# nidium/libapenetwork

Hardware: AMD Instinct MI355X
Metric: LZ4 GiB/s device-resident (compress+decompress), 1M×64KiB blocks, 1/2/4/8 GPU (higher is better)
Workload: dtype u8

## Files before the change

### libapenetwork_amd/csrc/lz4_encode.hip

```cpp
#include "lz4_gpu_internal.h"
#include <type_traits>

namespace apelz4 {

#ifdef APE_LZ4_STATS
__device__ unsigned long long g_enc_stats[16];
hipError_t enc_stats_read(unsigned long long *out, int reset) {
    hipError_t e = hipMemcpyFromSymbol(out, HIP_SYMBOL(g_enc_stats), sizeof(g_enc_stats));
    if (e == hipSuccess && reset) {
        unsigned long long z[16] = {0};
        e = hipMemcpyToSymbol(HIP_SYMBOL(g_enc_stats), z, sizeof(z));
    }
    return e;
}
#endif

namespace {

constexpr int kWavesPerEu = 7;

constexpr uint32_t kEagerLen = 12;
static_assert(kEagerLen + 4u == 16u, "in[T-4, T+kEagerLen) is one 16-byte load (loadv)");
constexpr uint32_t kEagerL = 12;
constexpr uint32_t kExt2 = 64;
constexpr uint32_t kGroups = 16;
constexpr uint32_t kRingE = 1024;
static_assert((kRingE & (kRingE - 1u)) == 0u && kRingE < 65536u,
              "the ring holds recent input, not the block's window (DESIGN.md 3.1.1)");
constexpr int kSmall = 128;
constexpr uint32_t kQ = 128;
constexpr uint32_t kFetchAt = 48, kEmitAll = 80, kChunkRecs = 64u / 4u;
static_assert((kQ & (kQ - 1u)) == 0u, "record ring indexed by & (kQ - 1)");
static_assert(kEmitAll - 1u + 2u * kChunkRecs <= kQ, "walker -> emitter record ring overflow");
static_assert(kFetchAt < kEmitAll, "a fetch precedes emit_all");
constexpr int kEmitEvery = 8;
constexpr uint32_t kStage = 512;
constexpr uint32_t kStageAlloc = kStage + 16u + 16u + 64u;


constexpr uint32_t I_TRUNC = 1u << 7, I_HASHABLE = 1u << 13;
static_assert(kEagerLen + kExt2 < 128u, "len fits 7 bits");

struct __attribute__((aligned(16))) EncLds {
    uint32_t ring[kRingE / 4 + 16];
    uint16_t tab[kHSize];
    uint2 info[64];
    uint2 q[kQ];
    uint32_t qn[2];
    uint8_t __attribute__((aligned(16))) stage[kStageAlloc];
};

template <int N>
__device__ __forceinline__ void vm_wait() {
    static_assert(N >= 0 && N < 16, "vmcnt");
    __builtin_amdgcn_s_waitcnt(N | (7 << 4) | (15 << 8));
}

__device__ __forceinline__ void shift_bytes(const uint32_t (&L)[8], int d, uint32_t (&X)[8]) {
    uint32_t T[8];
#pragma unroll
    for (int k = 0; k < 8; k++) T[k] = L[k];
    const bool down = d >= 0;
    const int ad = down ? d : -d, w = ad >> 2;
    const uint32_t r = (uint32_t)ad & 3u;
#pragma unroll
    for (int bit = 4; bit >= 1; bit >>= 1) {
        if (w & bit) {
            if (down) {
#pragma unroll
                for (int k = 0; k < 8; k++) T[k] = (k + bit < 8) ? T[k + bit] : 0u;
            } else {
#pragma unroll
                for (int k = 7; k >= 0; k--) T[k] = (k - bit >= 0) ? T[k - bit] : 0u;
            }
        }
    }
#pragma unroll
    for (int k = 0; k < 8; k++) {
        if (down) X[k] = __builtin_amdgcn_alignbyte(k + 1 < 8 ? T[k + 1] : 0u, T[k], r);
        else X[k] = r ? __builtin_amdgcn_alignbyte(T[k], k >= 1 ? T[k - 1] : 0u, 4u - r) : T[k];
    }
}

// ... 135 lines not shown
    int nch;
    int k0;
    uint32_t nr;
    uint32_t stride;
    gcu8 *win;
    uint32_t D;
};

template <bool EXT>
__device__ __forceinline__ gcu8 *hist(const Blk &B, uint32_t pos) {
    if constexpr (EXT) return pos < B.D ? B.win + pos : B.in + pos;
    else return B.in + pos;
}
template <bool EXT, int NA>
__device__ __forceinline__ void loadv_h(const Blk &B, uint32_t pos, uint32_t (&X)[NA], bool fast) {
    if constexpr (!EXT) {
        loadv(B.in, B.un, pos, X, fast);
    } else {
        gcu8 *q = hist<true>(B, pos);
        if (fast) {
            const uint4 a = gload16(q);
            X[0] = a.x; X[1] = a.y; X[2] = a.z; X[3] = a.w;
            return;
        }
#pragma unroll
        for (int k = 0; k < 4; k++) X[k] = 0;
#pragma unroll
        for (uint32_t t = 0; t < 16u; t++)
            if (pos + t < B.un) X[t >> 2] |= (uint32_t)q[t] << (8 * (t & 3));
    }
}

struct Part {
    uint32_t len, c, bk, lim, base;
    uint32_t iy;
    uint32_t rank, ntr, eo;
    bool hashable;
    uint64_t tmask;
    uint64_t smask;
};

struct PSet {
    uint32_t X[2];
    uint32_t Y[6];
    uint32_t E[4];
    uint32_t cT, jL, h;
    Part q;
};

template <bool SMALL, bool FAST = false, bool EXT = false>
__device__ __forceinline__ void prod_load(const Blk &B, int k, int lane, uint32_t (&X)[2]) {
    const uint32_t pos = (FAST || k < B.nch ? 64u * (uint32_t)k : (EXT ? B.D : 0u)) + (uint32_t)lane;
    if (FAST || (!SMALL && 64 * k + 72 <= B.n)) {
        const uint2 v = gload8(B.in + pos);
        X[0] = v.x;
        X[1] = v.y;
        return;
    }
    X[0] = X[1] = 0;
#pragma unroll
    for (uint32_t t = 0; t < 8u; t++)
        if (pos + t < B.un) X[t >> 2] |= (uint32_t)B.in[pos + t] << (8 * (t & 3));
}

template <bool SMALL, bool FAST = false, bool EXT = false>
__device__ __forceinline__ void prod_fetch_t(const Blk &B, int k, int lane, uint32_t cT,
                                             uint32_t (&Y)[6]) {
    const uint32_t p = 64u * (uint32_t)k + (uint32_t)lane;
    if (FAST) {
        loadv_h<EXT>(B, __builtin_elementwise_sub_sat(umin(cT, p - 1u), 4u), Y, true);
        return;
    }
    const bool tryT = k < B.nch && cT < p && cT >= 4u;
    loadv_h<EXT>(B, tryT ? cT - 4u : 0u, Y, !SMALL && 64 * k + 83 <= B.n);
}

template <bool SMALL, bool FAST = false, bool EXT = false>
__device__ __forceinline__ void prod_lookup(EncLds &S, const Blk &B, int k, int lane,
                                            const uint32_t (&X)[2], uint32_t &cT, uint32_t &jL,
                                            uint32_t &h, uint32_t (&Y)[6]) {
    const uint32_t p = 64u * (uint32_t)k + (uint32_t)lane;
    const bool hashable = FAST || (k < B.nch && p + 5u <= B.un);
    h = hashk(X[0], X[1]);
    cT = S.tab[h];
    jL = 0xFFFFFFFFu;
    if (hashable) S.tab[h] = (uint16_t)p;
    prod_fetch_t<SMALL, FAST, EXT>(B, k, lane, cT, Y);
}

template <bool FAST = false>
__device__ __forceinline__ void prod_ring(EncLds &S, const Blk &B, int k, int lane,
                                          const uint32_t (&X)[2]) {
    if (FAST || k < B.nch) {
        const uint32_t p = 64u * (uint32_t)k + (uint32_t)lane;
        const uint8_t by = (uint8_t)X[0];
        ((uint8_t *)S.ring)[p & (kRingE - 1)] = by;
        if (((64u * (uint32_t)k) & (kRingE - 1)) == 0u) ((uint8_t *)S.ring)[kRingE + lane] = by;
    }
}

__device__ __forceinline__ void prod_own(const EncLds &S, int k, int lane, uint32_t (&X)[6]) {
    const uint32_t p = 64u * (uint32_t)k + (uint32_t)lane;
    const uint32_t *r = S.ring + (((p - 4u) >> 2) & (kRingE / 4 - 1));
    const uint32_t sh = p & 3u;
    uint32_t W[7];
#pragma unroll
    for (int t = 0; t < 7; t++) W[t] = r[t];
#pragma unroll
    for (int t = 0; t < 6; t++) X[t] = __builtin_amdgcn_alignbyte(W[t + 1], W[t], sh);
}

__device__ __forceinline__ bool stage2_group(const Part &R, int lane, uint32_t first, uint32_t p,
                                             uint32_t &cb, uint32_t &eo) {
    const uint32_t r = R.rank - first, i16 = 16u * ((uint32_t)lane & 3u);
    const bool push = lane_in(R.smask) && r < kGroups;
    const int tgt = (int)((push ? 4u * r : ((uint32_t)lane | 1u)) << 2);
    cb = dpp_z<0x00>((uint32_t)__builtin_amdgcn_ds_permute(tgt, (int)(R.c + R.base))) + i16;
    eo = dpp_z<0x00>((uint32_t)__builtin_amdgcn_ds_permute(tgt, (int)(p + R.base))) + i16;
    return first + ((uint32_t)lane >> 2) < R.ntr;
}

__device__ __forceinline__ uint32_t stage2_len(const EncLds &S, int lane, uint32_t eo,
                                               const uint32_t (&E)[4]) {
    const uint4 o = ring16(S, eo);
    const uint32_t O[4] = {o.x, o.y, o.z, o.w};
    const uint32_t li = 128u * ((uint32_t)lane & 3u);
    uint32_t d = umin(first_diff_bit<0>(O, E), 8u * kExt2 - li) + li;
    d = umin(d, dpp<0xB1>(0u, d));
    d = umin(d, dpp<0x4E>(0u, d));
    const uint32_t len = d >> 3;
    return eo + len;
}

template <bool SMALL, bool FAST = false, bool EXT = false>
__device__ __forceinline__ void prod_measure(EncLds &S, const Blk &B, int k, int lane,
                                             const uint32_t (&X)[6], const uint32_t (&Y)[6],
                                             uint32_t cT, uint32_t jL, uint32_t h, Part &R) {
    const uint32_t p = 64u * (uint32_t)k + (uint32_t)lane;
    const bool live = FAST || k < B.nch;
    R.hashable = FAST || (live && p + 5u <= B.un);
    const bool can = FAST || (live && p >= 1u && p <= B.mstart && B.n >= kMinLength);
    const uint32_t cL = 64u * (uint32_t)k + jL;
    uint32_t Z[4];
#pragma unroll
    for (int t = 0; t < 4; t++) Z[t] = bperm(X[t], jL);
    constexpr bool okL = false;
    const bool okT = can & (cT < p) & (cT >= 4u) & (Y[1] == X[1]) & (!EXT | (cT + 3u - B.D > 6u));
    R.lim = FAST ? 0xFFFFu : (can ? B.mlimit - p : 0u);
    if constexpr (EXT) R.lim = cT < B.D ? umin(R.lim, B.D - cT) : R.lim;
    const uint32_t eT = eager(X, Y);
    const uint32_t eL = (umin(first_diff_bit<2>(X, Z), 8u * (kEagerL - 4u)) >> 3) + 4u;
    const uint32_t lT = okT ? eT : 0u, lL = okL ? eL : 0u;
    const bool pickL = okL & (!okT | ((lT < kEagerL) & (lL >= lT)));
    R.c = pickL ? cL : cT;
    R.len = pickL ? lL : lT;
    R.base = pickL ? kEagerL : kEagerLen;
    if (FAST && !EXT) {
        R.tmask = wave_ballot(R.len >= R.base);
    } else {
        R.tmask = wave_ballot(R.len >= R.base) & wave_ballot(R.lim > R.base);
        R.len = umin(R.len, R.lim);
    }
    {
        const uint32_t key = (R.c - (uint32_t)lane) + (R.base << 24);
        const uint32_t keyn = dpp_z<kDppWaveShl1>(key);
        R.smask = R.tmask & ~((R.tmask >> 1) & wave_ballot(key == keyn));
    }
    R.bk = umin(back4(X[0], pickL ? Z[0] : Y[0]), R.c);
    R.iy = ((okT | okL) ? p - R.c : 0u) | (h << 16);
}

template <bool SMALL, bool FAST = false, bool EXT = false>
__device__ __forceinline__ void prod_stage2_issue(const EncLds &S, const Blk &B, int k, int lane,
                                                  Part &R, uint32_t (&E)[4]) {
    const uint32_t p = 64u * (uint32_t)k + (uint32_t)lane;
    const uint64_t tb = R.smask;
    R.ntr = (uint32_t)__popcll(tb);
    R.rank = lane_rank(tb);
    uint32_t cb;
    const bool ga = stage2_group(R, lane, 0u, p, cb, R.eo);
    loadv_h<EXT>(B, ga ? cb : 0u, E, FAST || (!SMALL && 64 * k + 148 <= B.n));
}

template <bool SMALL, bool FAST = false, bool EXT = false>
__device__ __forceinline__ void prod_finish(EncLds &S, const Blk &B, int k, int lane,
                                            const Part &R, const uint32_t (&E)[4]) {
    const uint32_t p = 64u * (uint32_t)k + (uint32_t)lane;
    uint32_t len = R.len;
    bool trunc = false;
    {
        uint32_t mine = bperm(stage2_len(S, lane, R.eo, E), 4u * R.rank);
        for (uint32_t first = kGroups; first < R.ntr; first += kGroups) {
            uint32_t cb, eo, E2[4];
            const bool ga = stage2_group(R, lane, first, p, cb, eo);
            loadv_h<EXT>(B, ga ? cb : 0u, E2, FAST || (!SMALL && 64 * k + 148 <= B.n));
            const uint32_t m2 = bperm(stage2_len(S, lane, eo, E2), 4u * (R.rank - first));
            if (R.rank - first < kGroups) mine = m2;
        }
        if (lane_in(R.tmask)) {
            const uint32_t cap = R.base + kExt2, full = mine - p;
            len = (FAST && !EXT) ? umin(full, cap) : umin(umin(full, cap), R.lim);
            trunc = full >= cap && ((FAST && !EXT) || R.lim > cap);
        }
    }
    S.info[lane] = make_uint2(len | (R.bk << 8) | (trunc ? I_TRUNC : 0u) |
                                  ((FAST || R.hashable) ? I_HASHABLE : 0u),
                              R.iy);
}

struct Walk {
    uint32_t q;
    uint32_t anchor;
};

struct Probe {
    uint32_t s0, s1, g0;
};
__device__ __forceinline__ Probe probe_regime(uint32_t P, uint32_t e0, uint32_t acc) {
    const uint32_t y0 = P > e0 + 2u ? P - e0 - 2u : 0u;
    uint32_t s = 0, g = acc;
    while (y0 > s + 64u * g) {
        s += 64u * g;
        g++;
    }
    Probe R;
    R.s0 = s;
    R.s1 = s + 64u * g;
    R.g0 = g;
    return R;
}
__device__ __forceinline__ bool probed(uint32_t d, bool far, const Probe &R, uint32_t acc) {
    const uint32_t y = d - 2u;
    const bool hi = far && y > R.s1;
    const uint32_t base = far ? (hi ? R.s1 : R.s0) : 0u;
    const uint32_t g = far ? (hi ? R.g0 + 1u : R.g0) : acc;
    return d <= 2u || (y - base) % g == 0u;
}

template <bool EXT = false>
__device__ __forceinline__ uint32_t extend_match(const Blk &B, uint32_t m, uint32_t cm, uint32_t L,
// ... 9 lines not shown
                const uint4 x = gload16(B.in + (m + kk)), y = gload16(hist<EXT>(B, cm + kk));
                xb[0] = x.x; xb[1] = x.y; xb[2] = x.z; xb[3] = x.w;
                yb[0] = y.x; yb[1] = y.y; yb[2] = y.z; yb[3] = y.w;
            } else {
#pragma unroll
                for (uint32_t t = 0; t < 16u; t++) {
                    if (m + kk + t < B.un) {
                        xb[t >> 2] |= (uint32_t)B.in[m + kk + t] << (8 * (t & 3));
                        yb[t >> 2] |= (uint32_t)*hist<EXT>(B, cm + kk + t) << (8 * (t & 3));
                    }
                }
            }
#pragma unroll
            for (int t = 3; t >= 0; t--) {
                const uint32_t e = xb[t] ^ yb[t];
                if (e) { d = 1; at = 4u * (uint32_t)t + (__builtin_ctz(e) >> 3); }
            }
        }
        const uint64_t bad = wave_ballot(d != 0 || kk >= lm);
        if (bad) {
            const int fl = __builtin_ctzll(bad);
            const uint32_t k2 = L + 16u * (uint32_t)fl;
            L = k2 >= lm ? lm : k2 + lane_val(at, fl);
            break;
        }
        L += 1024u;
    }
    return L > lm ? lm : L;
}

struct WalkOut {
    uint64_t members;
    uint32_t m_back, m_len, an;
    uint2 iv;
    uint32_t q0, Lf;
    uint2 e2v;
    uint32_t e2h;
    uint32_t pmv, pe;
};

#pragma clang diagnostic push
#pragma clang diagnostic ignored "-Winline-asm"
__device__ __forceinline__ void hop_chain(uint64_t Hm, uint32_t nxt, uint32_t &rel, uint64_t &M, uint32_t &j,
                                          uint32_t &pe, uint32_t &pmv) {
    uint64_t t;
    asm volatile(
        "1:\n\t"
        "s_lshr_b64 %[t], %[hm], %[rel]\n\t"
        "s_cmp_eq_u64 %[t], 0\n\t"
        "s_cbranch_scc1 2f\n\t"
        "s_ff1_i32_b64 %[j], %[t]\n\t"
        "s_add_u32 %[j], %[j], %[rel]\n\t"
        "s_bitset1_b64 %[m], %[j]\n\t"
        "s_mov_b32 m0, %[j]\n\t"
        "v_writelane_b32 %[pmv], %[pe], m0\n\t"
        "v_readlane_b32 %[rel], %[nxt], %[j]\n\t"
        "s_mov_b32 %[pe], %[rel]\n\t"
        "s_cmp_lt_u32 %[rel], 64\n\t"
        "s_cbranch_scc1 1b\n\t"
        "s_branch 3f\n"
        "2:\n\t"
        "s_mov_b32 %[rel], 64\n"
        "3:"
        : [rel] "+s"(rel), [m] "+s"(M), [j] "+s"(j), [t] "=&s"(t), [pe] "+s"(pe), [pmv] "+v"(pmv)
        : [hm] "s"(Hm), [nxt] "v"(nxt)
        : "scc", "m0");
}
#pragma clang diagnostic pop

template <bool ACC, bool EXT = false>
__device__ __forceinline__ void walk_chain(const EncLds &S, const Blk &B, int k, int lane, Walk &W,
                                           WalkOut &O) {
    const uint32_t P = 64u * (uint32_t)k;
    O.members = 0;
    O.m_back = O.m_len = O.an = 0;
    O.iv = S.info[lane];
    O.q0 = W.q;
    O.pe = W.anchor - P;
    O.Lf = O.iv.x & 0x7Fu;
    if (W.q >= P + 64u) return;
    const uint2 iv = O.iv;
    const uint64_t Hm = wave_ballot(O.Lf != 0u);
    const uint32_t Lh = iv.x & 0xFFu;
    uint32_t rel = W.q - P;
    uint64_t M = 0;
    if constexpr (!ACC) {
        const uint32_t nxt = (uint32_t)lane + (iv.x & 0x7Fu) + ((iv.x & 0x80u) << 1);
        uint32_t j = 0;
        hop_chain(Hm, nxt, rel, M, j, O.pe, O.pmv);
        while (__builtin_expect(rel >= 256u, 0)) {
            const uint32_t me = P + j;
            const uint32_t cm = me - (lane_val(iv.y, (int)j) & 0xFFFFu);
            const uint32_t Le = extend_match<EXT>(B, me, cm, rel - 256u - j, lane);
            if ((uint32_t)lane == j) O.Lf = Le;
            rel = j + Le;
            O.pe = rel;
            if (rel >= 64u) break;
            hop_chain(Hm, nxt, rel, M, j, O.pe, O.pmv);
        }
        O.members = M;
        W.q = P + rel;
        return;
    }
    const Probe R = probe_regime(P, W.anchor, B.stride);
    uint32_t e = W.anchor;
    bool far = true;
    for (;;) {
        const uint32_t x = P + (uint32_t)lane;
        const uint64_t pm = wave_ballot(x >= e && probed(x - e, far, R, B.stride));
        const uint64_t w = (Hm & pm) >> rel;
        if (w == 0) {
            rel = 64u;
            break;
        }
        const uint32_t j = rel + (uint32_t)__builtin_ctzll(w);
        const uint32_t h = lane_val(Lh, (int)j);
        M |= 1ull << j;
        if (h & 0x80u) {
            const uint32_t me = P + j;
            const uint32_t cm = me - (lane_val(iv.y, (int)j) & 0xFFFFu);
            const uint32_t Le = extend_match<EXT>(B, me, cm, h & 0x7Fu, lane);
            if ((uint32_t)lane == j) O.Lf = Le;
            rel = j + Le;
        } else {
            rel = j + h;
        }
        e = P + rel;
        far = false;
        if (rel >= 64u) break;
    }
    O.members = M;
    W.q = P + rel;
}

template <bool ACC>
__device__ __forceinline__ void walk_finish(const Blk &B, int k, int lane, Walk &W, WalkOut &O) {
    const uint32_t P = 64u * (uint32_t)k;
    const uint32_t anchor0 = W.anchor;
    const bool mem = lane_in(O.members);
    const uint32_t p = P + (uint32_t)lane;
    uint32_t pm, lastend;
    if constexpr (!ACC) {
        pm = P + O.pmv;
        lastend = P + O.pe;
    } else {
        const uint32_t end = mem ? p + O.Lf : 0u;
        const uint32_t imax = wave_incl_max(end);
        pm = umax(wave_shr1(imax, 0u), anchor0);
        lastend = umax(anchor0, lane_val(imax, 63));
    }
    uint32_t bk = umin((O.iv.x >> 8) & 7u, p - pm);
    if (ACC) {
        const uint32_t c = p - (O.iv.y & 0xFFFFu);
        const uint32_t room = umin(p - pm, c);
        if (mem && bk == 4u && room > 4u) {
            const uint32_t lim = umin(room - 4u, 16u);
            uint32_t more = 0;
            for (uint32_t t = 1; t <= lim; t++) {
                if (B.in[p - 4u - t] != B.in[c - 4u - t]) break;
                more = t;
            }
            bk += more;
        }
    }
    O.m_back = bk;
    O.m_len = O.Lf + bk;
    O.an = pm;
    W.anchor = lastend;
}

__device__ __forceinline__ void walk_publish(EncLds &S, const Blk &B, int k, int lane,
                                             const WalkOut &O, uint32_t &qn) {
    const uint32_t p = 64u * (uint32_t)k + (uint32_t)lane;
    const uint2 iv = O.iv;
    const bool mem = lane_in(O.members);
    if (mem) S.q[(qn + lane_rank(O.members)) & (kQ - 1u)] =
        make_uint2(((p - O.m_back) - O.an) | ((O.m_len - kMinMatch) << 16), iv.y & 0xFFFFu);
    qn += (uint32_t)__popcll(O.members);
    if (lane == 0) S.qn[0] = qn;
}

struct Emit {
    uint32_t o;
    uint32_t ein;
    uint32_t qc;
    int last;
    bool overflow;
    bool part;
    int pend;
    bool nv;
    uint32_t o0, tot;
    uint64_t bigm;
    uint32_t r, lit, mlm4, off, ba;
};

__device__ __forceinline__ void stage_put(EncLds &S, int lane, bool w, uint32_t at, uint32_t b) {
    S.stage[w ? at : kStageAlloc - 64u + (uint32_t)lane] = (uint8_t)b;
}

__device__ __forceinline__ void emit_fetch(EncLds &S, const Blk &B, int lane, Emit &E,
                                           uint32_t avail, uint32_t rlo) {
    const bool v0 = (uint32_t)lane < avail;
    const uint2 rec = S.q[(E.qc + (uint32_t)lane) & (kQ - 1u)];
    const uint32_t lit = v0 ? (rec.x & 0xFFFFu) : 0u, mlm4 = v0 ? (rec.x >> 16) : 0u;
    const uint32_t size = v0 ? 3u + ext_bytes(lit) + lit + ext_bytes(mlm4) : 0u;
    const uint32_t isz = wave_incl_sum(size);
    const uint32_t nrec = umax((uint32_t)__popcll(wave_ballot(v0) & wave_ballot(isz <= kStage)), 1u);
    const bool v = (uint32_t)lane < nrec;
    const uint32_t adv = v ? lit + mlm4 + kMinMatch : 0u;
    const uint32_t iadv = wave_incl_sum(adv);
    const uint32_t tot = lane_val(isz, (int)nrec - 1), tadv = lane_val(iadv, (int)nrec - 1);
    E.qc += nrec;
// ... 123 lines not shown
        uint2 x[kU];
        bool ok[kU];
#pragma unroll
        for (int u = 0; u < kU; u++) {
            const uint32_t v = v0 + 192u * u + 3u * (uint32_t)lane;
            ok[u] = v < D && v + 8u <= B.un;
            x[u] = gload8(B.in + (ok[u] ? v : 0u));
        }
#pragma unroll
        for (int u = 0; u < kU; u++) {
            const uint32_t v = v0 + 192u * u + 3u * (uint32_t)lane;
            if (ok[u]) S.tab[hashk(x[u].x, x[u].y)] = (uint16_t)v;
        }
    }
    const uint32_t p = D - 64u + (uint32_t)lane;
    const uint8_t by = B.in[p];
    ((uint8_t *)S.ring)[p & (kRingE - 1)] = by;
    if (((D - 64u) & (kRingE - 1)) == 0u) ((uint8_t *)S.ring)[kRingE + lane] = by;
}

__device__ __forceinline__ void cdict_history(EncLds &S, const Blk &B, int lane) {
    const uint32_t p = B.D - 64u + (uint32_t)lane;
    const uint8_t by = B.win[p];
    ((uint8_t *)S.ring)[p & (kRingE - 1)] = by;
    if (((B.D - 64u) & (kRingE - 1)) == 0u) ((uint8_t *)S.ring)[kRingE + lane] = by;
}

template <bool SMALL, bool ACC, bool EXT = false>
__device__ __forceinline__ void encode_block(EncLds &S, const Blk &B, int wave, int lane,
                                             int *result, int *tail) {
    STATS_DECL
    const int k0 = B.k0;
    const int nch = B.nr >= (uint32_t)kMinLength ? B.nch : k0;
    const int nsteps = k0 + ((nch - k0 + 3) & ~1);

    if (wave == 1) {
        PSet P0, P1;
        auto pstep = [&](auto fast, int s, PSet &cur, PSet &nxt) {
            constexpr bool F = decltype(fast)::value;
            vm_wait<3>();
            STAT(9);
            prod_ring<F>(S, B, s + 2, lane, cur.X);
            uint32_t X6[6];
            prod_own(S, s + 1, lane, X6);
            prod_lookup<SMALL, F, EXT>(S, B, s + 2, lane, cur.X, cur.cT, cur.jL, cur.h, cur.Y);
            prod_load<SMALL, F, EXT>(B, s + 4, lane, cur.X);
            STAT(5);
            vm_wait<4>();
            STAT(9);
            prod_measure<SMALL, F, EXT>(S, B, s + 1, lane, X6, nxt.Y, nxt.cT, nxt.jL, nxt.h, nxt.q);
            STAT(5);
            __syncthreads();
            STAT(6);
            prod_stage2_issue<SMALL, F, EXT>(S, B, s + 1, lane, nxt.q, nxt.E);
            STAT(7);
            vm_wait<3>();
            STAT(9);
            prod_finish<SMALL, F, EXT>(S, B, s, lane, cur.q, cur.E);
            STAT(7);
            __syncthreads();
            STAT(8);
        };
        if constexpr (EXT) {
            if (k0 > 0) cdict_history(S, B, lane);
        } else {
            if (k0 > 0) prefix_history(S, B, lane);
        }
        if (nch > k0) {
            prod_load<SMALL, false, EXT>(B, k0, lane, P0.X);
            prod_load<SMALL, false, EXT>(B, k0 + 1, lane, P1.X);
            prod_ring(S, B, k0, lane, P0.X);
            prod_lookup<SMALL, false, EXT>(S, B, k0, lane, P0.X, P0.cT, P0.jL, P0.h, P0.Y);
            prod_load<SMALL, false, EXT>(B, k0 + 2, lane, P0.X);
            prod_ring(S, B, k0 + 1, lane, P1.X);
            prod_lookup<SMALL, false, EXT>(S, B, k0 + 1, lane, P1.X, P1.cT, P1.jL, P1.h, P1.Y);
            prod_load<SMALL, false, EXT>(B, k0 + 3, lane, P1.X);
            prod_ring(S, B, k0 + 2, lane, P0.X);
            uint32_t X6[6];
            prod_own(S, k0, lane, X6);
            prod_measure<SMALL, false, EXT>(S, B, k0, lane, X6, P0.Y, P0.cT, P0.jL, P0.h, P0.q);
            prod_stage2_issue<SMALL, false, EXT>(S, B, k0, lane, P0.q, P0.E);
        }
        __builtin_amdgcn_s_waitcnt(0);
        __syncthreads();
        constexpr int kFastEnd = 328;
        const int nfast_abs = SMALL ? 0 : (int)umin((uint32_t)(B.n >= kFastEnd ? (B.n - kFastEnd) / 64 + 1 : 0),
                                                    (uint32_t)nsteps);
        const int nfast = nfast_abs > k0 ? k0 + ((nfast_abs - k0) & ~1) : k0;
        int s = k0;
        for (; s < nfast; s += 2) {
            pstep(std::true_type{}, s, P0, P1);
            pstep(std::true_type{}, s + 1, P1, P0);
        }
        for (; s < nsteps; s += 2) {
            pstep(std::false_type{}, s, P0, P1);
            pstep(std::false_type{}, s + 1, P1, P0);
        }
        STATS_FLUSH_TID(g_enc_stats, 64);
        return;
    }
    if (wave == 0) {
        Walk W;
        uint32_t qn = 0;
        W.q = 64u * (uint32_t)k0;
        W.anchor = W.q;
        WalkOut O;
        __syncthreads();
        const int s2 = nch + 1;
        __syncthreads();
        __syncthreads();
        int s = k0 + 1;
        for (; s < s2; s++) {
            walk_chain<ACC, EXT>(S, B, s - 1, lane, W, O);
            STAT(0);
            __syncthreads();
            STAT(4);
            walk_finish<ACC>(B, s - 1, lane, W, O);
            walk_publish(S, B, s - 1, lane, O, qn);
            STAT_ADD(11, __popcll(O.members));
            STAT(1);
            STAT_ADD(10, 3);
            __syncthreads();
            STAT(3);
        }
        for (; s < nsteps; s++) {
            __syncthreads();
            __syncthreads();
        }
        STATS_FLUSH(g_enc_stats);
        return;
    }
    Emit E;
    E.o = 0;
    E.ein = 64u * (uint32_t)k0;
    E.qc = 0;
    E.last = k0;
    E.overflow = false;
    E.part = false;
    E.pend = 0;
    E.nv = false;
    E.o0 = E.tot = 0;
    E.bigm = 0;
    E.r = E.lit = E.mlm4 = E.off = E.ba = 0;
    __syncthreads();
    for (int s = k0; s < nsteps; s++) {
        const uint32_t qr = (uint32_t)__builtin_amdgcn_readfirstlane(S.qn[0]);
        const uint32_t avail = umax(qr, E.qc) - E.qc;
        if (E.pend == 0) {
            if (avail != 0u && (avail >= kFetchAt || s - E.last >= kEmitEvery)) {
                emit_fetch(S, B, lane, E, avail, s >= 12 ? 64u * (uint32_t)(s - 12) : 0u);
                E.last = s;
            }
        } else if (avail >= kEmitAll) {
            emit_all(S, B, lane, E);
        } else {
            emit_step(S, B, lane, E);
        }
        STAT(2);
        __syncthreads();
        STAT(14);
        if (E.pend == 1 || E.pend == 3) emit_step(S, B, lane, E);
        STAT(12);
        __syncthreads();
        STAT(15);
    }
    emit_all(S, B, lane, E);
    {
        const uint32_t rlo = B.nch > 16 ? 64u * (uint32_t)(B.nch - 16) : 0u;
        for (uint32_t left = (uint32_t)__builtin_amdgcn_readfirstlane(umax(S.qn[0], S.qn[1])) - E.qc; left;) {
            const uint32_t qc0 = E.qc;
            emit_fetch(S, B, lane, E, left, rlo);
            emit_all(S, B, lane, E);
            left -= E.qc - qc0;
        }
    }
    if (!E.overflow) emit_tail(S, B, lane, E);
    uint32_t last_run = 0;
    if (!E.overflow) {
        const uint32_t anchor = E.ein;
        const uint32_t lit = B.un - anchor;
        last_run = lit;
        const uint32_t hdr = 1u + ext_bytes(lit);
        const uint32_t total = E.o + hdr + lit;
        if (total > B.cap) {
            E.overflow = true;
        } else {
            if (lane == 0) {
                B.dst[E.o] = (uint8_t)((lit < 15u ? lit : 15u) << 4);
                put_len(B.dst + E.o + 1, lit);
            }
            wave_copy(B.in, B.dst, anchor, E.o + hdr, lit, lane);
            E.o = total;
        }
    }
    if (lane == 0) {
        *result = E.overflow ? 0 : (int)E.o;
        if (tail) *tail = E.overflow ? 0 : (int)last_run;
    }
    STAT_ADD(13, 1);
    STATS_FLUSH_TID(g_enc_stats, 128);
}

// ... 5 lines not shown
    __shared__ EncLds S;
    const int b = blockIdx.x;
    const int tid = threadIdx.x;
    const int lane = tid & 63, wave = __builtin_amdgcn_readfirstlane(tid >> 6);

    Blk B;
    B.in = (gcu8 *)(a.src ? a.src[b] : a.src_base + (size_t)b * a.src_stride);
    B.dst = (gu8 *)(a.dst ? a.dst[b] : a.dst_base + (size_t)b * a.dst_stride);
    const int nr = a.src_size[b];
    const int icap = a.dst_cap ? a.dst_cap[b] : (int)a.dst_stride;
    if (nr < 0 || nr > kMaxBlock || icap < 0) {
        if (tid == 0) a.result[b] = (nr > kMaxBlock) ? kErange : 0;
        return;
    }
    int D = 0;
    if (a.dict_size) {
        const int pre = a.dict_size[b];
        D = (pre > 0 ? (pre < kMaxBlock - nr ? pre : kMaxBlock - nr) : 0) & ~63;
        if (D < 64) D = 0;
    }
    B.in -= D;
    B.n = D + nr;
    B.nr = (uint32_t)nr;
    B.k0 = D / 64;
    B.stride = ACC ? (a.accel < (1 << 20) ? (uint32_t)a.accel : 1u << 20) : 1u;
    B.cap = (uint32_t)icap;
    B.un = (uint32_t)B.n;
    B.mstart = B.un >= 12 ? B.un - 12 : 0;
    B.mlimit = B.un >= 5 ? B.un - 5 : 0;
    B.nch = (B.n + 63) / 64;

    for (int i = tid; i < kHSize / 8; i += 192) ((uint4 *)S.tab)[i] = make_uint4(0, 0, 0, 0);
    for (int i = tid; i < (int)(kRingE / 16 + 4); i += 192) ((uint4 *)S.ring)[i] = make_uint4(0, 0, 0, 0);
    if (tid == 0) S.qn[0] = S.qn[1] = 0u;
    __syncthreads();
    int *const tail = a.tail ? a.tail + b : nullptr;
    if (B.n < kSmall) encode_block<true, ACC>(S, B, wave, lane, &a.result[b], tail);
    else encode_block<false, ACC>(S, B, wave, lane, &a.result[b], tail);
}

__global__ void __launch_bounds__(192) __attribute__((amdgpu_waves_per_eu(kWavesPerEu)))
lz4_encode_cdict_kernel(BlockArgs a, const uint8_t *cd) {
    __shared__ EncLds S;
    const int b = blockIdx.x;
    const int tid = threadIdx.x;
    const int lane = tid & 63, wave = __builtin_amdgcn_readfirstlane(tid >> 6);

    const CDictHdr H = *(const CDictHdr *)cd;
    if (H.magic != kCdMagic || H.D > kCdMaxWin || (H.D & 63u) != 0u || H.max_src < 1u ||
        H.max_src > (uint32_t)kMaxBlock || H.D + H.max_src > (uint32_t)kMaxBlock) {
        if (tid == 0) a.result[b] = 0;
        return;
    }
    const int nr = a.src_size[b];
    const int icap = a.dst_cap[b];
    if (nr < 0 || nr > (int)H.max_src || icap < 0) {
        if (tid == 0) a.result[b] = (nr > (int)H.max_src) ? kErange : 0;
        return;
    }
    const int D = (int)H.D;
    Blk B;
    B.win = (gcu8 *)(cd + kCdWin + kCdFront);
    B.D = (uint32_t)D;
    B.in = (gcu8 *)a.src[b] - D;
    B.dst = (gu8 *)a.dst[b];
    B.n = D + nr;
    B.nr = (uint32_t)nr;
    B.k0 = D / 64;
    B.stride = 1u;
    B.cap = (uint32_t)icap;
    B.un = (uint32_t)B.n;
    B.mstart = B.un >= 12 ? B.un - 12 : 0;
    B.mlimit = B.un >= 5 ? B.un - 5 : 0;
    B.nch = (B.n + 63) / 64;

    const uint4 *img = (const uint4 *)(cd + kCdTab);
    for (int i = tid; i < kHSize / 8; i += 192) ((uint4 *)S.tab)[i] = img[i];
    for (int i = tid; i < (int)(kRingE / 16 + 4); i += 192) ((uint4 *)S.ring)[i] = make_uint4(0, 0, 0, 0);
    if (tid == 0) S.qn[0] = S.qn[1] = 0u;
    __syncthreads();
    if (B.n < kSmall) encode_block<true, false, true>(S, B, wave, lane, &a.result[b], nullptr);
    else encode_block<false, false, true>(S, B, wave, lane, &a.result[b], nullptr);
}

hipError_t launch_encode_cdict(const BlockArgs &a, const void *cdict, hipStream_t s) {
    if (a.nblocks <= 0) return hipSuccess;
    hipLaunchKernelGGL(lz4_encode_cdict_kernel, dim3(a.nblocks), dim3(192), 0, s, a,
                       (const uint8_t *)cdict);
    return hipGetLastError();
}

hipError_t launch_encode(const BlockArgs &a, hipStream_t s) {
    if (a.nblocks <= 0) return hipSuccess;
    if (a.accel > 1)
        hipLaunchKernelGGL(lz4_encode_kernel<true>, dim3(a.nblocks), dim3(192), 0, s, a);
    else
        hipLaunchKernelGGL(lz4_encode_kernel<false>, dim3(a.nblocks), dim3(192), 0, s, a);
    return hipGetLastError();
}

}
```

Before: 148.0.

## Batch match-length stage-2 over chunk pairs and pack per-lane match info into one word

The producer wave now measures two 64-byte chunks before issuing the stage-2 match-extension loads, so candidates from both chunks share one set of 16-group ds_permute/load passes instead of one pass per chunk. Per-lane match info (offset, length, back-extension, trunc, hashable) is packed into a single 32-bit word in a double-buffered info array. Dead lazy-match code and the second qn counter are removed, and the schedule arithmetic moves into a shared constexpr header. This aims to cut permute and load overhead and register pressure in the encoder pipeline, at the cost of extra latency per pair and more complex barrier bookkeeping between producer, walker and emitter waves.

```diff
diff --git a/libapenetwork_amd/csrc/lz4_enc_sched.h b/libapenetwork_amd/csrc/lz4_enc_sched.h
--- /dev/null
+++ b/libapenetwork_amd/csrc/lz4_enc_sched.h
@@ -0,0 +1,74 @@
+#ifndef APE_LZ4_ENC_SCHED_H
+#define APE_LZ4_ENC_SCHED_H
+
+#if defined(__HIPCC__) || defined(__CUDACC__)
+#define APE_SCHED_FN __host__ __device__ constexpr
+#else
+#define APE_SCHED_FN constexpr
+#endif
+
+namespace apelz4 {
+namespace sched {
+
+constexpr int kRingChunks = 16;
+constexpr int kPrologue = -1;
+
+struct At {
+    int step, half;
+};
+
+APE_SCHED_FN int imax(int a, int b) { return a > b ? a : b; }
+
+APE_SCHED_FN int nchunks(int nch, int k0) { return nch > k0 ? nch - k0 : 0; }
+
+APE_SCHED_FN int enc_nsteps(int nch, int k0) { return k0 + ((nchunks(nch, k0) + 3) & ~1); }
+
+APE_SCHED_FN int pair_first(int k, int k0) { return k - ((k - k0) & 1); }
+APE_SCHED_FN int info_slot(int k, int k0) { return (k - k0) & 1; }
+
+APE_SCHED_FN At at_ring(int k, int k0) { return At{k - 2 > k0 ? k - 2 : k0 + kPrologue, 0}; }
+APE_SCHED_FN At at_lookup(int k, int k0) { return At{imax(k - 2, k0 + kPrologue), 0}; }
+APE_SCHED_FN At at_load(int k, int k0) { return At{imax(k - 4, k0 + kPrologue), 0}; }
+APE_SCHED_FN At at_measure(int k, int k0) { return At{imax(k - 1, k0 + kPrologue), 0}; }
+APE_SCHED_FN At at_s2_issue(int k, int k0) { return At{pair_first(k, k0), 1}; }
+APE_SCHED_FN At at_finish(int k, int k0) { return At{pair_first(k, k0) + 1, 1}; }
+APE_SCHED_FN At at_walk(int k, int) { return At{k + 2, 0}; }
+APE_SCHED_FN At at_publish(int k, int) { return At{k + 2, 1}; }
+
+APE_SCHED_FN int prod_begin(int, int k0) { return k0; }
+APE_SCHED_FN int prod_end(int nch, int k0) { return enc_nsteps(nch, k0); }
+constexpr int kFastBytes = 328;
+APE_SCHED_FN int prod_fast_end(int n, int nch, int k0, bool small) {
+    const int lim = small || n < kFastBytes ? 0 : (n - kFastBytes) / 64 + 1;
+    const int abs_end = lim < enc_nsteps(nch, k0) ? lim : enc_nsteps(nch, k0);
+    return abs_end > k0 ? k0 + ((abs_end - k0) & ~1) : k0;
+}
+APE_SCHED_FN int walk_begin(int, int k0) { return k0 + 2; }
+APE_SCHED_FN int walk_end(int nch, int k0) { return k0 + 2 + nchunks(nch, k0); }
+APE_SCHED_FN int walk_chunk(int s) { return s - 2; }
+APE_SCHED_FN int emit_begin(int, int k0) { return k0; }
+APE_SCHED_FN int emit_end(int nch, int k0) { return enc_nsteps(nch, k0); }
+
+APE_SCHED_FN int prod_barriers(int nch, int k0) {
+    return 1 + 2 * (prod_end(nch, k0) - prod_begin(nch, k0));
+}
+APE_SCHED_FN int walk_barriers(int nch, int k0) {
+    return 1 + 2 * (walk_begin(nch, k0) - k0) + 2 * (walk_end(nch, k0) - walk_begin(nch, k0)) +
+           2 * (enc_nsteps(nch, k0) - walk_end(nch, k0));
+}
+APE_SCHED_FN int emit_barriers(int nch, int k0) {
+    return 1 + 2 * (emit_end(nch, k0) - emit_begin(nch, k0));
+}
+
+APE_SCHED_FN int ring_hi(int s, int nch) { return s + 2 < nch - 1 ? s + 2 : nch - 1; }
+APE_SCHED_FN int ring_lo(int s, int nch) { return imax(ring_hi(s, nch) - (kRingChunks - 1), 0); }
+APE_SCHED_FN int emit_ring_bound(int s) { return imax(s - 12, 0); }
+APE_SCHED_FN int emit_tail_bound(int nch) { return imax(nch - kRingChunks, 0); }
+
+APE_SCHED_FN int measure_reach(int k) { return k + 1; }
+APE_SCHED_FN int finish_reach(int k) { return k + 2; }
+
+}
+}
+
+#endif
diff --git a/libapenetwork_amd/csrc/lz4_encode.hip b/libapenetwork_amd/csrc/lz4_encode.hip
--- a/libapenetwork_amd/csrc/lz4_encode.hip
+++ b/libapenetwork_amd/csrc/lz4_encode.hip
@@ -1,4 +1,5 @@
 #include "lz4_gpu_internal.h"
+#include "lz4_enc_sched.h"
 #include <type_traits>
 
 namespace apelz4 {
@@ -21,7 +22,6 @@
 
 constexpr uint32_t kEagerLen = 12;
 static_assert(kEagerLen + 4u == 16u, "in[T-4, T+kEagerLen) is one 16-byte load (loadv)");
-constexpr uint32_t kEagerL = 12;
 constexpr uint32_t kExt2 = 64;
 constexpr uint32_t kGroups = 16;
 constexpr uint32_t kRingE = 1024;
@@ -38,17 +38,19 @@
 constexpr uint32_t kStageAlloc = kStage + 16u + 16u + 64u;
 
 
-constexpr uint32_t I_TRUNC = 1u << 7, I_HASHABLE = 1u << 13;
+constexpr uint32_t I_LEN = 16, I_TRUNC = 1u << 23, I_BACK = 24, I_HASHABLE = 1u << 27;
 static_assert(kEagerLen + kExt2 < 128u, "len fits 7 bits");
 
 struct __attribute__((aligned(16))) EncLds {
     uint32_t ring[kRingE / 4 + 16];
     uint16_t tab[kHSize];
-    uint2 info[64];
+    uint32_t info[2][64];
     uint2 q[kQ];
-    uint32_t qn[2];
+    uint32_t qn;
     uint8_t __attribute__((aligned(16))) stage[kStageAlloc];
 };
+static_assert(sizeof(EncLds) <= 17904, "the block's LDS (DESIGN.md 3.1)");
+static_assert(9 * sizeof(EncLds) <= 160 * 1024, "9 blocks per CU");
 
 template <int N>
 __device__ __forceinline__ void vm_wait() {
@@ -250,20 +252,23 @@
 }
 
 struct Part {
-    uint32_t len, c, bk, lim, base;
-    uint32_t iy;
-    uint32_t rank, ntr, eo;
-    bool hashable;
+    uint32_t w;
+    uint32_t lim;
     uint64_t tmask;
     uint64_t smask;
 };
 
+struct Pass {
+    uint32_t E[4];
+    uint32_t eo;
+    uint32_t E2[4], eo2;
+    uint32_t n0, ntr;
+};
+
 struct PSet {
     uint32_t X[2];
     uint32_t Y[6];
-    uint32_t E[4];
-    uint32_t cT, jL, h;
-    Part q;
+    uint32_t cT;
 };
 
 template <bool SMALL, bool FAST = false, bool EXT = false>
@@ -295,13 +300,12 @@
 
 template <bool SMALL, bool FAST = false, bool EXT = false>
 __device__ __forceinline__ void prod_lookup(EncLds &S, const Blk &B, int k, int lane,
-                                            const uint32_t (&X)[2], uint32_t &cT, uint32_t &jL,
-                                            uint32_t &h, uint32_t (&Y)[6]) {
+                                            const uint32_t (&X)[2], uint32_t &cT,
+                                            uint32_t (&Y)[6]) {
     const uint32_t p = 64u * (uint32_t)k + (uint32_t)lane;
     const bool hashable = FAST || (k < B.nch && p + 5u <= B.un);
-    h = hashk(X[0], X[1]);
+    const uint32_t h = hashk(X[0], X[1]);
     cT = S.tab[h];
-    jL = 0xFFFFFFFFu;
     if (hashable) S.tab[h] = (uint16_t)p;
     prod_fetch_t<SMALL, FAST, EXT>(B, k, lane, cT, Y);
 }
@@ -328,14 +332,26 @@
     for (int t = 0; t < 6; t++) X[t] = __builtin_amdgcn_alignbyte(W[t + 1], W[t], sh);
 }
 
-__device__ __forceinline__ bool stage2_group(const Part &R, int lane, uint32_t first, uint32_t p,
-                                             uint32_t &cb, uint32_t &eo) {
-    const uint32_t r = R.rank - first, i16 = 16u * ((uint32_t)lane & 3u);
-    const bool push = lane_in(R.smask) && r < kGroups;
-    const int tgt = (int)((push ? 4u * r : ((uint32_t)lane | 1u)) << 2);
-    cb = dpp_z<0x00>((uint32_t)__builtin_amdgcn_ds_permute(tgt, (int)(R.c + R.base))) + i16;
-    eo = dpp_z<0x00>((uint32_t)__builtin_amdgcn_ds_permute(tgt, (int)(p + R.base))) + i16;
-    return first + ((uint32_t)lane >> 2) < R.ntr;
+__device__ __forceinline__ uint32_t rank_a(const Part &A) { return lane_rank(A.smask); }
+__device__ __forceinline__ uint32_t rank_b(const Part &Bp, uint32_t n0) {
+    return __builtin_amdgcn_mbcnt_hi((uint32_t)(Bp.smask >> 32),
+                                     __builtin_amdgcn_mbcnt_lo((uint32_t)Bp.smask, n0));
+}
+
+__device__ __forceinline__ bool stage2_group(const Part &A, const Part &Bp, int lane, uint32_t first,
+                                             uint32_t pa, uint32_t ra, uint32_t rb, uint32_t n0,
+                                             uint32_t ntr, uint32_t &cb, uint32_t &eo) {
+    const uint32_t i16 = 16u * ((uint32_t)lane & 3u), idle = ((uint32_t)lane | 1u) << 2;
+    const uint32_t qa = ra - first, qb = rb - first;
+    const int ta = (int)((lane_in(A.smask) && qa < kGroups) ? 16u * qa : idle);
+    const int tb = (int)((lane_in(Bp.smask) && qb < kGroups) ? 16u * qb : idle);
+    const uint32_t va = (uint32_t)__builtin_amdgcn_ds_permute(ta, (int)((A.w & 0xFFFFu) | (pa << 16)));
+    const uint32_t vb = (uint32_t)__builtin_amdgcn_ds_permute(tb, (int)((Bp.w & 0xFFFFu) | ((pa + 64u) << 16)));
+    const uint32_t g = first + ((uint32_t)lane >> 2);
+    const uint32_t v = dpp_z<0x00>(g < n0 ? va : vb);
+    eo = (v >> 16) + (kEagerLen + i16);
+    cb = eo - (v & 0xFFFFu);
+    return g < ntr;
 }
 
 __device__ __forceinline__ uint32_t stage2_len(const EncLds &S, int lane, uint32_t eo,
@@ -353,77 +369,84 @@
 template <bool SMALL, bool FAST = false, bool EXT = false>
 __device__ __forceinline__ void prod_measure(EncLds &S, const Blk &B, int k, int lane,
                                              const uint32_t (&X)[6], const uint32_t (&Y)[6],
-                                             uint32_t cT, uint32_t jL, uint32_t h, Part &R) {
+                                             uint32_t cT, Part &R) {
     const uint32_t p = 64u * (uint32_t)k + (uint32_t)lane;
     const bool live = FAST || k < B.nch;
-    R.hashable = FAST || (live && p + 5u <= B.un);
+    const bool hashable = FAST || (live && p + 5u <= B.un);
     const bool can = FAST || (live && p >= 1u && p <= B.mstart && B.n >= kMinLength);
-    const uint32_t cL = 64u * (uint32_t)k + jL;
-    uint32_t Z[4];
-#pragma unroll
-    for (int t = 0; t < 4; t++) Z[t] = bperm(X[t], jL);
-    constexpr bool okL = false;
     const bool okT = can & (cT < p) & (cT >= 4u) & (Y[1] == X[1]) & (!EXT | (cT + 3u - B.D > 6u));
     R.lim = FAST ? 0xFFFFu : (can ? B.mlimit - p : 0u);
     if constexpr (EXT) R.lim = cT < B.D ? umin(R.lim, B.D - cT) : R.lim;
     const uint32_t eT = eager(X, Y);
-    const uint32_t eL = (umin(first_diff_bit<2>(X, Z), 8u * (kEagerL - 4u)) >> 3) + 4u;
-    const uint32_t lT = okT ? eT : 0u, lL = okL ? eL : 0u;
-    const bool pickL = okL & (!okT | ((lT < kEagerL) & (lL >= lT)));
-    R.c = pickL ? cL : cT;
-    R.len = pickL ? lL : lT;
-    R.base = pickL ? kEagerL : kEagerLen;
+    uint32_t len = okT ? eT : 0u;
     if (FAST && !EXT) {
-        R.tmask = wave_ballot(R.len >= R.base);
+        R.tmask = wave_ballot(len >= kEagerLen);
     } else {
-        R.tmask = wave_ballot(R.len >= R.base) & wave_ballot(R.lim > R.base);
-        R.len = umin(R.len, R.lim);
+        R.tmask = wave_ballot(len >= kEagerLen) & wave_ballot(R.lim > kEagerLen);
+        len = umin(len, R.lim);
     }
     {
-        const uint32_t key = (R.c - (uint32_t)lane) + (R.base << 24);
+        const uint32_t key = cT - (uint32_t)lane;
         const uint32_t keyn = dpp_z<kDppWaveShl1>(key);
         R.smask = R.tmask & ~((R.tmask >> 1) & wave_ballot(key == keyn));
     }
-    R.bk = umin(back4(X[0], pickL ? Z[0] : Y[0]), R.c);
-    R.iy = ((okT | okL) ? p - R.c : 0u) | (h << 16);
+    const uint32_t bk = umin(back4(X[0], Y[0]), cT);
+    R.w = (okT ? p - cT : 0u) | (len << I_LEN) | (bk << I_BACK) | (hashable ? I_HASHABLE : 0u);
 }
 
 template <bool SMALL, bool FAST = false, bool EXT = false>
 __device__ __forceinline__ void prod_stage2_issue(const EncLds &S, const Blk &B, int k, int lane,
-                                                  Part &R, uint32_t (&E)[4]) {
-    const uint32_t p = 64u * (uint32_t)k + (uint32_t)lane;
-    const uint64_t tb = R.smask;
-    R.ntr = (uint32_t)__popcll(tb);
-    R.rank = lane_rank(tb);
+                                                  const Part &A, const Part &Bp, Pass &Q) {
+    const uint32_t pa = 64u * (uint32_t)k + (uint32_t)lane;
+    Q.n0 = (uint32_t)__popcll(A.smask);
+    Q.ntr = Q.n0 + (uint32_t)__popcll(Bp.smask);
+    const uint32_t ra = rank_a(A), rb = rank_b(Bp, Q.n0);
+    const bool inside = FAST || (!SMALL && 64 * (k + 1) + 148 <= B.n);
     uint32_t cb;
-    const bool ga = stage2_group(R, lane, 0u, p, cb, R.eo);
-    loadv_h<EXT>(B, ga ? cb : 0u, E, FAST || (!SMALL && 64 * k + 148 <= B.n));
+    const bool ga = stage2_group(A, Bp, lane, 0u, pa, ra, rb, Q.n0, Q.ntr, cb, Q.eo);
+    loadv_h<EXT>(B, ga ? cb : 0u, Q.E, inside);
+    if (Q.ntr > kGroups) {
+        const bool gb = stage2_group(A, Bp, lane, kGroups, pa, ra, rb, Q.n0, Q.ntr, cb, Q.eo2);
+        loadv_h<EXT>(B, gb ? cb : 0u, Q.E2, inside);
+    }
+}
+
+template <bool FAST, bool EXT>
+__device__ __forceinline__ uint32_t finish_word(const Part &R, uint32_t mine, uint32_t p) {
+    uint32_t w = R.w;
+    if (lane_in(R.tmask)) {
+        const uint32_t cap = kEagerLen + kExt2, full = mine - p;
+        const uint32_t len = (FAST && !EXT) ? umin(full, cap) : umin(umin(full, cap), R.lim);
+        const bool trunc = full >= cap && ((FAST && !EXT) || R.lim > cap);
+        w = (w & ~(0xFFu << I_LEN)) | (len << I_LEN) | (trunc ? I_TRUNC : 0u);
+    }
+    return w;
 }
 
 template <bool SMALL, bool FAST = false, bool EXT = false>
 __device__ __forceinline__ void prod_finish(EncLds &S, const Blk &B, int k, int lane,
-                                            const Part &R, const uint32_t (&E)[4]) {
-    const uint32_t p = 64u * (uint32_t)k + (uint32_t)lane;
-    uint32_t len = R.len;
-    bool trunc = false;
-    {
-        uint32_t mine = bperm(stage2_len(S, lane, R.eo, E), 4u * R.rank);
-        for (uint32_t first = kGroups; first < R.ntr; first += kGroups) {
-            uint32_t cb, eo, E2[4];
-            const bool ga = stage2_group(R, lane, first, p, cb, eo);
-            loadv_h<EXT>(B, ga ? cb : 0u, E2, FAST || (!SMALL && 64 * k + 148 <= B.n));
-            const uint32_t m2 = bperm(stage2_len(S, lane, eo, E2), 4u * (R.rank - first));
-            if (R.rank - first < kGroups) mine = m2;
-        }
-        if (lane_in(R.tmask)) {
-            const uint32_t cap = R.base + kExt2, full = mine - p;
-            len = (FAST && !EXT) ? umin(full, cap) : umin(umin(full, cap), R.lim);
-            trunc = full >= cap && ((FAST && !EXT) || R.lim > cap);
-        }
-    }
-    S.info[lane] = make_uint2(len | (R.bk << 8) | (trunc ? I_TRUNC : 0u) |
-                                  ((FAST || R.hashable) ? I_HASHABLE : 0u),
-                              R.iy);
+                                            const Part &A, const Part &Bp, const Pass &Q) {
+    const uint32_t pa = 64u * (uint32_t)k + (uint32_t)lane;
+    const uint32_t ra = rank_a(A), rb = rank_b(Bp, Q.n0);
+    const uint32_t g0 = stage2_len(S, lane, Q.eo, Q.E);
+    uint32_t ma = bperm(g0, 4u * ra), mb = bperm(g0, 4u * rb);
+    if (Q.ntr > kGroups) {
+        const uint32_t g1 = stage2_len(S, lane, Q.eo2, Q.E2);
+        const uint32_t a1 = bperm(g1, 4u * (ra - kGroups)), b1 = bperm(g1, 4u * (rb - kGroups));
+        if (ra - kGroups < kGroups) ma = a1;
+        if (rb - kGroups < kGroups) mb = b1;
+    }
+    for (uint32_t first = 2u * kGroups; first < Q.ntr; first += kGroups) {
+        uint32_t cb, eo, E2[4];
+        const bool ga = stage2_group(A, Bp, lane, first, pa, ra, rb, Q.n0, Q.ntr, cb, eo);
+        loadv_h<EXT>(B, ga ? cb : 0u, E2, FAST || (!SMALL && 64 * (k + 1) + 148 <= B.n));
+        const uint32_t g2 = stage2_len(S, lane, eo, E2);
+        const uint32_t a2 = bperm(g2, 4u * (ra - first)), b2 = bperm(g2, 4u * (rb - first));
+        if (ra - first < kGroups) ma = a2;
+        if (rb - first < kGroups) mb = b2;
+    }
+    S.info[0][lane] = finish_word<FAST, EXT>(A, ma, pa);
+    S.info[1][lane] = finish_word<FAST, EXT>(Bp, mb, pa + 64u);
 }
 
 struct Walk {
@@ -499,10 +522,8 @@
 struct WalkOut {
     uint64_t members;
     uint32_t m_back, m_len, an;
-    uint2 iv;
-    uint32_t q0, Lf;
-    uint2 e2v;
-    uint32_t e2h;
+    uint32_t iv;
+    uint32_t Lf;
     uint32_t pmv, pe;
 };
 
@@ -536,28 +557,27 @@
 #pragma clang diagnostic pop
 
 template <bool ACC, bool EXT = false>
-__device__ __forceinline__ void walk_chain(const EncLds &S, const Blk &B, int k, int lane, Walk &W,
-                                           WalkOut &O) {
+__device__ __forceinline__ void walk_chain(const EncLds &S, const Blk &B, int k, int slot, int lane,
+                                           Walk &W, WalkOut &O) {
     const uint32_t P = 64u * (uint32_t)k;
     O.members = 0;
     O.m_back = O.m_len = O.an = 0;
-    O.iv = S.info[lane];
-    O.q0 = W.q;
+    O.iv = S.info[slot][lane];
     O.pe = W.anchor - P;
-    O.Lf = O.iv.x & 0x7Fu;
+    const uint32_t iv = O.iv;
+    const uint32_t Lh = (iv >> I_LEN) & 0xFFu;
+    O.Lf = Lh & 0x7Fu;
     if (W.q >= P + 64u) return;
-    const uint2 iv = O.iv;
     const uint64_t Hm = wave_ballot(O.Lf != 0u);
-    const uint32_t Lh = iv.x & 0xFFu;
     uint32_t rel = W.q - P;
     uint64_t M = 0;
     if constexpr (!ACC) {
-        const uint32_t nxt = (uint32_t)lane + (iv.x & 0x7Fu) + ((iv.x & 0x80u) << 1);
+        const uint32_t nxt = (uint32_t)lane + Lh + (Lh & 0x80u);
         uint32_t j = 0;
         hop_chain(Hm, nxt, rel, M, j, O.pe, O.pmv);
         while (__builtin_expect(rel >= 256u, 0)) {
             const uint32_t me = P + j;
-            const uint32_t cm = me - (lane_val(iv.y, (int)j) & 0xFFFFu);
+            const uint32_t cm = me - (lane_val(iv, (int)j) & 0xFFFFu);
             const uint32_t Le = extend_match<EXT>(B, me, cm, rel - 256u - j, lane);
             if ((uint32_t)lane == j) O.Lf = Le;
             rel = j + Le;
@@ -585,7 +605,7 @@
         M |= 1ull << j;
         if (h & 0x80u) {
             const uint32_t me = P + j;
-            const uint32_t cm = me - (lane_val(iv.y, (int)j) & 0xFFFFu);
+            const uint32_t cm = me - (lane_val(iv, (int)j) & 0xFFFFu);
             const uint32_t Le = extend_match<EXT>(B, me, cm, h & 0x7Fu, lane);
             if ((uint32_t)lane == j) O.Lf = Le;
             rel = j + Le;
@@ -616,9 +636,9 @@
         pm = umax(wave_shr1(imax, 0u), anchor0);
         lastend = umax(anchor0, lane_val(imax, 63));
     }
-    uint32_t bk = umin((O.iv.x >> 8) & 7u, p - pm);
+    uint32_t bk = umin((O.iv >> I_BACK) & 7u, p - pm);
     if (ACC) {
-        const uint32_t c = p - (O.iv.y & 0xFFFFu);
+        const uint32_t c = p - (O.iv & 0xFFFFu);
         const uint32_t room = umin(p - pm, c);
         if (mem && bk == 4u && room > 4u) {
             const uint32_t lim = umin(room - 4u, 16u);
@@ -639,12 +659,11 @@
 __device__ __forceinline__ void walk_publish(EncLds &S, const Blk &B, int k, int lane,
                                              const WalkOut &O, uint32_t &qn) {
     const uint32_t p = 64u * (uint32_t)k + (uint32_t)lane;
-    const uint2 iv = O.iv;
     const bool mem = lane_in(O.members);
     if (mem) S.q[(qn + lane_rank(O.members)) & (kQ - 1u)] =
-        make_uint2(((p - O.m_back) - O.an) | ((O.m_len - kMinMatch) << 16), iv.y & 0xFFFFu);
+        make_uint2(((p - O.m_back) - O.an) | ((O.m_len - kMinMatch) << 16), O.iv & 0xFFFFu);
     qn += (uint32_t)__popcll(O.members);
-    if (lane == 0) S.qn[0] = qn;
+    if (lane == 0) S.qn = qn;
 }
 
 struct Emit {
@@ -834,31 +853,44 @@
     STATS_DECL
     const int k0 = B.k0;
     const int nch = B.nr >= (uint32_t)kMinLength ? B.nch : k0;
-    const int nsteps = k0 + ((nch - k0 + 3) & ~1);
+    const int nsteps = sched::enc_nsteps(nch, k0);
 
     if (wave == 1) {
         PSet P0, P1;
-        auto pstep = [&](auto fast, int s, PSet &cur, PSet &nxt) {
+        Part QA, QB, QN;
+        Pass QP;
+        QA.w = QA.lim = 0u;
+        QA.tmask = QA.smask = 0;
+        auto phalf = [&](auto fast, auto yw, int s, PSet &cur, PSet &nxt, Part &out) {
             constexpr bool F = decltype(fast)::value;
             vm_wait<3>();
             STAT(9);
             prod_ring<F>(S, B, s + 2, lane, cur.X);
             uint32_t X6[6];
             prod_own(S, s + 1, lane, X6);
-            prod_lookup<SMALL, F, EXT>(S, B, s + 2, lane, cur.X, cur.cT, cur.jL, cur.h, cur.Y);
+            prod_lookup<SMALL, F, EXT>(S, B, s + 2, lane, cur.X, cur.cT, cur.Y);
             prod_load<SMALL, F, EXT>(B, s + 4, lane, cur.X);
             STAT(5);
-            vm_wait<4>();
+            vm_wait<decltype(yw)::value>();
             STAT(9);
-            prod_measure<SMALL, F, EXT>(S, B, s + 1, lane, X6, nxt.Y, nxt.cT, nxt.jL, nxt.h, nxt.q);
+            prod_measure<SMALL, F, EXT>(S, B, s + 1, lane, X6, nxt.Y, nxt.cT, out);
             STAT(5);
             __syncthreads();
             STAT(6);
-            prod_stage2_issue<SMALL, F, EXT>(S, B, s + 1, lane, nxt.q, nxt.E);
+        };
+        auto ppair = [&](auto fast, int f) {
+            constexpr bool F = decltype(fast)::value;
+            phalf(fast, std::integral_constant<int, 3>{}, f, P0, P1, QB);
+            prod_stage2_issue<SMALL, F, EXT>(S, B, f, lane, QA, QB, QP);
             STAT(7);
-            vm_wait<3>();
+            __syncthreads();
+            STAT(8);
+            phalf(fast, std::integral_constant<int, 4>{}, f + 1, P1, P0, QN);
+            STAT(7);
+            vm_wait<2>();
             STAT(9);
-            prod_finish<SMALL, F, EXT>(S, B, s, lane, cur.q, cur.E);
+            prod_finish<SMALL, F, EXT>(S, B, f, lane, QA, QB, QP);
+            QA = QN;
             STAT(7);
             __syncthreads();
             STAT(8);
@@ -872,32 +904,22 @@
             prod_load<SMALL, false, EXT>(B, k0, lane, P0.X);
             prod_load<SMALL, false, EXT>(B, k0 + 1, lane, P1.X);
             prod_ring(S, B, k0, lane, P0.X);
-            prod_lookup<SMALL, false, EXT>(S, B, k0, lane, P0.X, P0.cT, P0.jL, P0.h, P0.Y);
+            prod_lookup<SMALL, false, EXT>(S, B, k0, lane, P0.X, P0.cT, P0.Y);
             prod_load<SMALL, false, EXT>(B, k0 + 2, lane, P0.X);
             prod_ring(S, B, k0 + 1, lane, P1.X);
-            prod_lookup<SMALL, false, EXT>(S, B, k0 + 1, lane, P1.X, P1.cT, P1.jL, P1.h, P1.Y);
+            prod_lookup<SMALL, false, EXT>(S, B, k0 + 1, lane, P1.X, P1.cT, P1.Y);
             prod_load<SMALL, false, EXT>(B, k0 + 3, lane, P1.X);
             prod_ring(S, B, k0 + 2, lane, P0.X);
             uint32_t X6[6];
             prod_own(S, k0, lane, X6);
-            prod_measure<SMALL, false, EXT>(S, B, k0, lane, X6, P0.Y, P0.cT, P0.jL, P0.h, P0.q);
-            prod_stage2_issue<SMALL, false, EXT>(S, B, k0, lane, P0.q, P0.E);
+            prod_measure<SMALL, false, EXT>(S, B, k0, lane, X6, P0.Y, P0.cT, QA);
         }
         __builtin_amdgcn_s_waitcnt(0);
         __syncthreads();
-        constexpr int kFastEnd = 328;
-        const int nfast_abs = SMALL ? 0 : (int)umin((uint32_t)(B.n >= kFastEnd ? (B.n - kFastEnd) / 64 + 1 : 0),
-                                                    (uint32_t)nsteps);
-        const int nfast = nfast_abs > k0 ? k0 + ((nfast_abs - k0) & ~1) : k0;
-        int s = k0;
-        for (; s < nfast; s += 2) {
-            pstep(std::true_type{}, s, P0, P1);
-            pstep(std::true_type{}, s + 1, P1, P0);
-        }
-        for (; s < nsteps; s += 2) {
-            pstep(std::false_type{}, s, P0, P1);
-            pstep(std::false_type{}, s + 1, P1, P0);
-        }
+        const int nfast = sched::prod_fast_end(B.n, nch, k0, SMALL);
+        int s = sched::prod_begin(nch, k0);
+        for (; s < nfast; s += 2) ppair(std::true_type{}, s);
+        for (; s < sched::prod_end(nch, k0); s += 2) ppair(std::false_type{}, s);
         STATS_FLUSH_TID(g_enc_stats, 64);
         return;
     }
@@ -908,17 +930,19 @@
         W.anchor = W.q;
         WalkOut O;
         __syncthreads();
-        const int s2 = nch + 1;
-        __syncthreads();
-        __syncthreads();
-        int s = k0 + 1;
-        for (; s < s2; s++) {
-            walk_chain<ACC, EXT>(S, B, s - 1, lane, W, O);
+        int s = k0;
+        for (; s < sched::walk_begin(nch, k0); s++) {
+            __syncthreads();
+            __syncthreads();
+        }
+        for (; s < sched::walk_end(nch, k0); s++) {
+            const int k = sched::walk_chunk(s);
+            walk_chain<ACC, EXT>(S, B, k, sched::info_slot(k, k0), lane, W, O);
             STAT(0);
             __syncthreads();
             STAT(4);
-            walk_finish<ACC>(B, s - 1, lane, W, O);
-            walk_publish(S, B, s - 1, lane, O, qn);
+            walk_finish<ACC>(B, k, lane, W, O);
+            walk_publish(S, B, k, lane, O, qn);
             STAT_ADD(11, __popcll(O.members));
             STAT(1);
             STAT_ADD(10, 3);
@@ -945,12 +969,12 @@
     E.bigm = 0;
     E.r = E.lit = E.mlm4 = E.off = E.ba = 0;
     __syncthreads();
-    for (int s = k0; s < nsteps; s++) {
-        const uint32_t qr = (uint32_t)__builtin_amdgcn_readfirstlane(S.qn[0]);
+    for (int s = sched::emit_begin(nch, k0); s < sched::emit_end(nch, k0); s++) {
+        const uint32_t qr = (uint32_t)__builtin_amdgcn_readfirstlane(S.qn);
         const uint32_t avail = umax(qr, E.qc) - E.qc;
         if (E.pend == 0) {
             if (avail != 0u && (avail >= kFetchAt || s - E.last >= kEmitEvery)) {
-                emit_fetch(S, B, lane, E, avail, s >= 12 ? 64u * (uint32_t)(s - 12) : 0u);
+                emit_fetch(S, B, lane, E, avail, 64u * (uint32_t)sched::emit_ring_bound(s));
                 E.last = s;
             }
         } else if (avail >= kEmitAll) {
@@ -968,8 +992,8 @@
     }
     emit_all(S, B, lane, E);
     {
-        const uint32_t rlo = B.nch > 16 ? 64u * (uint32_t)(B.nch - 16) : 0u;
-        for (uint32_t left = (uint32_t)__builtin_amdgcn_readfirstlane(umax(S.qn[0], S.qn[1])) - E.qc; left;) {
+        const uint32_t rlo = 64u * (uint32_t)sched::emit_tail_bound(B.nch);
+        for (uint32_t left = (uint32_t)__builtin_amdgcn_readfirstlane(S.qn) - E.qc; left;) {
             const uint32_t qc0 = E.qc;
             emit_fetch(S, B, lane, E, left, rlo);
             emit_all(S, B, lane, E);
@@ -1041,7 +1065,7 @@
 
     for (int i = tid; i < kHSize / 8; i += 192) ((uint4 *)S.tab)[i] = make_uint4(0, 0, 0, 0);
     for (int i = tid; i < (int)(kRingE / 16 + 4); i += 192) ((uint4 *)S.ring)[i] = make_uint4(0, 0, 0, 0);
-    if (tid == 0) S.qn[0] = S.qn[1] = 0u;
+    if (tid == 0) S.qn = 0u;
     __syncthreads();
     int *const tail = a.tail ? a.tail + b : nullptr;
     if (B.n < kSmall) encode_block<true, ACC>(S, B, wave, lane, &a.result[b], tail);
@@ -1086,7 +1110,7 @@
     const uint4 *img = (const uint4 *)(cd + kCdTab);
     for (int i = tid; i < kHSize / 8; i += 192) ((uint4 *)S.tab)[i] = img[i];
     for (int i = tid; i < (int)(kRingE / 16 + 4); i += 192) ((uint4 *)S.ring)[i] = make_uint4(0, 0, 0, 0);
-    if (tid == 0) S.qn[0] = S.qn[1] = 0u;
+    if (tid == 0) S.qn = 0u;
     __syncthreads();
     if (B.n < kSmall) encode_block<true, false, true>(S, B, wave, lane, &a.result[b], nullptr);
     else encode_block<false, false, true>(S, B, wave, lane, &a.result[b], nullptr);
```

Result: no change. 148.5 (median of 6 runs) (+0.4%).
